# njspix/frender

Measured on AMD Instinct MI355X. Metric: M reads/sec scanned+classified (96 samples, 8+8bp, n=1) at 1/2/4/8 MI355X, higher is better.
Workload: dtype u8; 1 GPU; BASELINE config 2: 100000000 SYN-v1 reads/GPU, 96 samples, 8+8bp, n=1, R=8 (74 B/record), decoded FASTQ resident in HBM; reads_per_gpu=100000000, bytes_per_record=74, samples=96, nsubs=1, rc=False, unique_codes=1383958, table_checksum=a89b0e2c6adb2921, parallelism=1 GPU

## Files before the change

### frender_amd/csrc/fr_kernels.hip

```cpp
#include <algorithm>
#include <cstdlib>
#include <cstring>

#include <rocprim/rocprim.hpp>

#include "../../include/frender_amd.h"
#include "fr_internal.h"

namespace fr {

#if defined(FR_STAMPS) && FR_STAMPS == 1
#define FR_STAMP_DECL u64 st_[8] = {0, 0, 0, 0, 0, 0, 0, 0}; u64 tq_ = __builtin_amdgcn_s_memtime();
#define FR_STAMP(i) do { const u64 n_ = __builtin_amdgcn_s_memtime(); st_[i] += n_ - tq_; tq_ = n_; } while (0)
#define FR_STAMP_FLUSH(k0) do { st_[6] = __builtin_amdgcn_s_memtime() - (k0); \
    if ((threadIdx.x & 63) == 0) for (int i_ = 0; i_ < 8; ++i_) atomicAdd((unsigned long long*)&a.st->stamp[i_], \
        (unsigned long long)st_[i_]); } while (0)
#else
#define FR_STAMP_DECL
#define FR_STAMP(i) do { } while (0)
#define FR_STAMP_FLUSH(k0) do { } while (0)
#endif

#if defined(FR_STAMPS) && FR_STAMPS == 2
#define FR_CSTAMP(i) do { const u64 n_ = __builtin_amdgcn_s_memtime(); cst_[i] += n_ - cq_; cq_ = n_; } while (0)
#else
#define FR_CSTAMP(i) do { } while (0)
#endif

#if defined(FR_STAMPS) && FR_STAMPS == 4
#define FR_WSTAMP_DECL u64 wst_[4] = {0, 0, 0, 0}; u64 wq_ = __builtin_amdgcn_s_memtime();
#define FR_WSTAMP(i) do { const u64 n_ = __builtin_amdgcn_s_memtime(); wst_[i] += n_ - wq_; wq_ = n_; } while (0)
#define FR_WSTAMP_RESET() do { wq_ = __builtin_amdgcn_s_memtime(); } while (0)
#define FR_WSTAMP_FLUSH(steps) do { if ((threadIdx.x & 63) == 0) { \
    for (int i_ = 0; i_ < 4; ++i_) atomicAdd((unsigned long long*)&a.st->stamp[i_], (unsigned long long)wst_[i_]); \
    atomicAdd((unsigned long long*)&a.st->stamp[4], (unsigned long long)(steps)); \
    atomicAdd((unsigned long long*)&a.st->stamp[6], 1ull); } } while (0)
#else
#define FR_WSTAMP_DECL
#define FR_WSTAMP(i) do { } while (0)
#define FR_WSTAMP_RESET() do { } while (0)
#define FR_WSTAMP_FLUSH(steps) do { } while (0)
#endif

#ifdef FR_DEBUG_PRINT
#define FR_TRACE(...) do { if (blockIdx.x == 0 && (threadIdx.x & 63) == 0) printf(__VA_ARGS__); } while (0)
#else
#define FR_TRACE(...) do { } while (0)
#endif

#define FR_COLD __forceinline__

#ifndef FR_ABLATE
#define FR_ABLATE 0
#endif
constexpr u32 ABLATE = FR_ABLATE;


__device__ __forceinline__ u32 eq4(u32 w, u32 c) {
    const u32 t = w ^ c;
    const u32 z = ~(((t & 0x7F7F7F7Fu) + 0x7F7F7F7Fu) | t) & 0x80808080u;
    return (((z >> 7) * 0x00204081u) >> 21) & 0xFu;
}

__device__ __forceinline__ u32 hi4(u32 w) {
    return ((((w & 0x80808080u) >> 7) * 0x00204081u) >> 21) & 0xFu;
}

__device__ __forceinline__ u32 sym_of(u32 c) {
    const u32 i = (c >> 1) & 7u;
    const u64 expect = 0x4E002B0047544341ull;
    const u32 symtab = 0x50603421u;
    const bool ok = ((expect >> (8 * i)) & 0xFFu) == c;
    return ok ? ((symtab >> (4 * i)) & 0xFu) : 0u;
}

__device__ __forceinline__ u32 classify4(u32 w) {
    const u32 lo3 = __builtin_amdgcn_perm(0x10101310u, 0x10191014u, w & 0x07070707u);
    const u32 mid3 = __builtin_amdgcn_perm(0x18101014u, 0x10101310u, (w >> 3) & 0x07070707u);
    const u32 top2 = __builtin_amdgcn_perm(0u, 0x1010000Fu, (w >> 6) & 0x03030303u);
    return lo3 & mid3 & top2;
}

__device__ __forceinline__ u32 classify4_fast(u32 w) {
    const u32 lo3 = __builtin_amdgcn_perm(0x00008300u, 0x00890084u, w & 0x07070707u);
    const u32 hi4 = __builtin_amdgcn_perm(0x08000004u, 0x00000300u, (w >> 3) & 0x0F0F0F0Fu);
    return lo3 & hi4;
}

template <int K>
__device__ __forceinline__ u32 gather16(u32 c0, u32 c1, u32 c2, u32 c3) {
    constexpr u32 M = 0x01010101u << K;
    u32 v = __builtin_amdgcn_udot4(c0 & M, 0x08040201u, 0u, false);
    v = __builtin_amdgcn_udot4(c1 & M, 0x80402010u, v, false);
    u32 u = __builtin_amdgcn_udot4(c2 & M, 0x08040201u, 0u, false);
    u = __builtin_amdgcn_udot4(c3 & M, 0x80402010u, u, false);
    return (v | (u << 8)) >> K;
}

#ifndef FR_CLS_PAIR
#define FR_CLS_PAIR 1
#endif

constexpr u32 PAIR_CR = 0x04040404u, PAIR_SENTINEL = 0x40404040u;
__device__ __forceinline__ u32 classify8_pair(u32 wa, u32 wb) {
    const u32 lo_a = __builtin_amdgcn_perm(0x00004500u, 0x00430048u, wa & 0x87878787u);
    const u32 hi_a = __builtin_amdgcn_perm(0x02000008u, 0x00000500u, (wa >> 3) & 0x1F1F1F1Fu);
    const u32 lo_b = __builtin_amdgcn_perm(0x00005400u, 0x007000C0u, wb & 0x87878787u);
    const u32 hi_b = __builtin_amdgcn_perm(0x20000080u, 0x00001400u, (wb >> 3) & 0x1F1F1F1Fu);
    return __builtin_amdgcn_bitop3_b32(lo_a, hi_a, lo_b & hi_b, 0xEAu);
}

template <int K>
__device__ __forceinline__ u32 gather16p(u32 d0, u32 d1) {
    constexpr u32 M = 0x11111111u << K;
    const u32 v = __builtin_amdgcn_udot4(d0 & M, 0x08040201u, 0u, false);
    const u32 u = __builtin_amdgcn_udot4(d1 & M, 0x08040201u, 0u, false);
    return v | (u << 8);
}

template <int K>
__device__ __forceinline__ u64 join16p(const u32 (&g)[4]) {
    const u32 lo = (g[0] >> K) | (g[1] << (16 - K)), hi = (g[2] >> K) | (g[3] << (16 - K));
    return ((u64)hi << 32) | (u64)lo;
}

__device__ __forceinline__ u64 agent_load(const u64* p) {
    return __hip_atomic_load(p, __ATOMIC_RELAXED, __HIP_MEMORY_SCOPE_AGENT);
}
__device__ __forceinline__ void agent_store(u64* p, u64 v) {
    __hip_atomic_store(p, v, __ATOMIC_RELAXED, __HIP_MEMORY_SCOPE_AGENT);
}

__device__ __forceinline__ u64 wave_sum_u64(u64 v) {
#pragma unroll
    for (int d = 32; d >= 1; d >>= 1) v += __shfl_xor(v, d, 64);
    return v;
}

__device__ __forceinline__ u64 table_home(u64 key, u64 mask) {
    return mask ? mix64(key) >> __builtin_clzll(mask) : 0ull;
}

__device__ bool global_insert(const Table& T, DevState* st, u64 key, u64 cnt, u64 ord, u32 tag) {
    u64 h = table_home(key, T.mask);
    for (int probe = 0; probe < GPROBE; ++probe) {
        GSlot* s = &T.slots[h];
        const uint4 w0 = *(const uint4*)s;
        const uint4 w1 = *((const uint4*)s + 1);
        u64 k = ((u64)w0.y << 32) | w0.x;
        u64 first = ((u64)w1.y << 32) | w1.x;
        u32 ltag = w1.z;
        bool created = false;
        if (k == 0) {
            const u64 old = atomicCAS((unsigned long long*)&s->key, 0ull, (unsigned long long)key);
            created = old == 0;
            k = created ? key : old;
            first = ~0ull;
            ltag = 0;
        }
        if (k == key) {
            atomicAdd((unsigned long long*)&s->count, (unsigned long long)cnt);
            if (ord < first) atomicMin((unsigned long long*)&s->first, (unsigned long long)ord);
            if (ltag < tag) atomicMax(&s->last_tag, tag);
            return created;
        }
        h = (h + 1) & T.mask;
    }
    const u64 i = atomicAdd((unsigned long long*)&st->n_overflow, 1ull);
    if (i < T.ovf_cap) {
        Overflow o;
        o.key = key;
        o.count = cnt;
        o.first = ord;
        o.tag = tag;
        o.pad = 0;
        T.ovf[i] = o;
    } else {
        atomicOr(&st->cap_flags, 2u);
    }
    return false;
}

__device__ __forceinline__ void add_created(DevState* st, u32 mine) {
    u64 v = mine;
#pragma unroll
    for (int d = 32; d >= 1; d >>= 1) v += __shfl_xor(v, d, 64);
    if ((threadIdx.x & 63) == 0 && v) atomicAdd((unsigned long long*)&st->n_keys, (unsigned long long)v);
}

struct alignas(16) LSlot {
    u64 key;
    u32 cnt;
    u32 mino;
};

constexpr int NW = WG / 64;
constexpr int SEGS = TILE / SEG;
constexpr u32 RARE_WAVE = RARE_RING / NW;

struct ScanShared {
    u32 raw[NW][TILE / 4];
    LSlot ls[NS];
    u64 bsp[NW][SEGS + 2];
    u64 bcol[NW][SEGS + 2];
    u64 beol[NW][SEGS + 2];
    u64 wcount[NW];
    int wphase[NW];
    u32 rq_tail[NW];
    u64 tile_excl;
    u64 cbase;
    u32 chunk;
    u32 nkeys;
    u32 created;
    u32 flags;
    u32 last;
    u32 spec;
    u32 spec_bad;
    u32 ncold;
    u32 nexo;
    u32 err_off;
    u32 log_on;
    u32 exo_p[EXO_BUF], exo_start[EXO_BUF], exo_len[EXO_BUF];
};

typedef u32 u32x4 __attribute__((ext_vector_type(4)));
typedef __attribute__((address_space(3))) u32 lds_u32;
typedef __attribute__((address_space(3))) u32x4 lds_u32x4;
typedef __attribute__((address_space(3))) u64 lds_u64;
typedef __attribute__((address_space(3))) u8 lds_u8;

__device__ __forceinline__ u64 make_ord(const ScanArgs& a, u64 off_in_range) {
    return ((u64)a.file_tag << ORD_SHIFT) | ((a.file_offset + off_in_range) & ~3ull);
}

__device__ __forceinline__ u32 wave_id() { return __builtin_amdgcn_readfirstlane(threadIdx.x >> 6); }

__device__ __forceinline__ void lds_fence() {
    __builtin_amdgcn_fence(__ATOMIC_RELEASE, "workgroup", "local");
    __builtin_amdgcn_fence(__ATOMIC_ACQUIRE, "workgroup", "local");
}

__device__ __forceinline__ void lds_barrier() {
    __builtin_amdgcn_fence(__ATOMIC_RELEASE, "workgroup", "local");
    __builtin_amdgcn_s_barrier();
    __builtin_amdgcn_fence(__ATOMIC_ACQUIRE, "workgroup", "local");
}

__device__ FR_COLD void direct_insert(ScanShared& sh, const ScanArgs& a, u64 key, u32 off) {
    if (global_insert(a.tabv, a.st, key, 1, make_ord(a, sh.cbase + off), a.file_tag)) atomicAdd(&sh.created, 1u);
}

__device__ __forceinline__ void rare_push(ScanShared& sh, const ScanArgs& a, u32 p, u32 kind, u32 x, u32 y);

// ... 164 lines not shown
        if (c == '+') {
            if (plus != WIDE_NOPLUS) return false;
            plus = nl;
            continue;
        }
        const u32 lc = c | 0x20u;
        const int d = lc == 'a' ? 0 : lc == 'c' ? 1 : lc == 'g' ? 2 : lc == 't' ? 3 : lc == 'n' ? 4 : -1;
        if (d < 0 || nl >= WIDE_MAXN) return false;
        const int isl = (c & 0x20u) ? 1 : 0;
        if (lower < 0) lower = isl;
        else if (lower != isl) return false;
        v += (u64)d * pw;
        pw *= 5;
        ++nl;
    }
    if (lower < 0) return false;
    const int n1 = plus == WIDE_NOPLUS ? nl : plus, n2 = plus == WIDE_NOPLUS ? 0 : nl - plus;
    if (n1 > MAXSYM || n2 > MAXSYM) return false;
    key = WIDE_BIT | ((u64)lower << 62) | ((u64)plus << 57) | (v + (pw - 1) / 4);
    return true;
}

__device__ void exotic_record(const ScanArgs& a, u32 p, u64 start, u64 n, ScanShared& sh) {
    {
        bool fast = n >= 1 && n <= (u64)MAXSYM;
        u64 key = 0;
        for (u64 i = 0; fast && i < n; ++i) {
            const u32 sy = sym_of(a.buf[start + i]);
            fast = sy != 0;
            key |= (u64)sy << (3 * i);
        }
        if (fast || wide_encode(a, start, n, key)) {
            count_code<true>(sh, a, p, key);
            return;
        }
    }
    if (sh.spec) {
        const u32 k = atomicAdd(&sh.nexo, 1u);
        if (k < (u32)EXO_BUF) {
            sh.exo_p[k] = p;
            sh.exo_start[k] = (u32)(start - sh.cbase);
            sh.exo_len[k] = (u32)n;
        } else {
            atomicOr(&sh.spec_bad, 1u);
        }
        return;
    }
    const u64 i = atomicAdd((unsigned long long*)&a.st->n_exotic, 1ull);
    const u64 po = atomicAdd((unsigned long long*)&a.st->exo_pool_used, (unsigned long long)n);
    if (i < a.tabv.exo_cap && po + n <= a.tabv.exo_pool_cap) {
        a.tabv.exo_ord[i] = make_ord(a, sh.cbase + p);
        a.tabv.exo_off[i] = po;
        a.tabv.exo_len[i] = (u32)n;
        for (u64 k = 0; k < n; ++k) a.tabv.exo_pool[po + k] = a.buf[start + k];
    } else {
        atomicOr(&a.st->cap_flags, 4u);
    }
}

__device__ __forceinline__ void nospace(const ScanArgs& a, u32 p, ScanShared& sh) {
    if (sh.spec) atomicMin(&sh.err_off, p);
    else atomicMin((unsigned long long*)&a.st->err_nospace, (unsigned long long)(a.file_offset + sh.cbase + p));
}

__device__ FR_COLD void process_header_global(ScanShared& sh, const ScanArgs& a, u32 p) {
    const u64 eof = a.avail;
    auto rd = [&](u64 q) -> u32 { return (u32)a.buf[q]; };
    u64 q = sh.cbase + p;
    for (;;) {
        if (q >= eof) return nospace(a, p, sh);
        const u32 c = rd(q);
        if (c == ' ') break;
        if (c == '\n' || c == '\r') return nospace(a, p, sh);
        ++q;
    }
    const u64 sp1 = q++;
    i64 lc = -1;
    for (;;) {
        if (q >= eof) break;
        const u32 c = rd(q);
        if (c == ' ' || c == '\n' || c == '\r') break;
        if (c == ':') lc = (i64)q;
        ++q;
    }
    const u64 start = (lc >= 0 ? (u64)lc : sp1) + 1;
    const u64 n = q - start;
    u64 key = 0;
    bool fast = n >= 1 && n <= (u64)MAXSYM;
    for (u64 i = 0; fast && i < n; ++i) {
        const u32 sy = sym_of(rd(start + i));
        fast = sy != 0;
        key |= (u64)sy << (3 * i);
    }
    if (fast) count_code<true>(sh, a, p, key);
    else exotic_record(a, p, start, n, sh);
}

struct SegRegs {
    uint4 v[SEG / 16];
    u32 nx;
};

__device__ __forceinline__ void seg_fetch(const ScanArgs& a, u32 t, SegRegs& r, int lane, bool with_nx = false) {
    const u64 tile0 = (u64)t * TSTEP;
    const u32 nb = (u32)min((u64)TILE, a.avail - tile0);
    const u64 base = (u64)(a.buf + tile0);
    const u32 lo = __builtin_amdgcn_readfirstlane((u32)base), hi = __builtin_amdgcn_readfirstlane((u32)(base >> 32));
    const u8* ub = (const u8*)(((u64)hi << 32) | lo);
    const auto rsrc = __builtin_amdgcn_make_buffer_rsrc((void*)ub, (short)0, (int)__builtin_amdgcn_readfirstlane(nb),
                                                        0x00020000);
#pragma unroll
    for (int k = 0; k < SEG / 16; ++k) {
        const auto v = __builtin_amdgcn_raw_buffer_load_b128(rsrc, lane * SEG, k * 16, 0);
        r.v[k] = make_uint4(v[0], v[1], v[2], v[3]);
    }
    r.nx = with_nx ? __builtin_amdgcn_raw_buffer_load_b32(rsrc, lane * SEG + SEG, 0, 0) : 0u;
}

__device__ __attribute__((noinline)) SegRegs seg_load_tail(const ScanArgs& a, u32 t, int lane) {
    const u64 tile0 = (u64)t * TSTEP;
    const u32 nb = (u32)min((u64)TILE, a.avail - tile0);
    const u32 s0 = lane * SEG;
    u32 w[SEG / 4 + 1];
    for (int k = 0; k <= SEG / 4; ++k) {
        u32 v = 0;
        for (u32 q = 0; q < 4; ++q) {
            const u32 o = s0 + 4 * k + q;
            if (o < nb) v |= (u32)a.buf[tile0 + o] << (8 * q);
        }
        w[k] = v;
    }
    SegRegs r;
    for (int k = 0; k < SEG / 16; ++k) r.v[k] = make_uint4(w[4 * k], w[4 * k + 1], w[4 * k + 2], w[4 * k + 3]);
    r.nx = w[SEG / 4];
    return r;
}

__device__ __forceinline__ bool seg_in_range(const ScanArgs& a, u32 t) {
    return (u64)t * TSTEP + (TILE + SEG + 4) <= a.avail;
}

__device__ __forceinline__ void seg_load(const ScanArgs& a, u32 t, SegRegs& r, int lane) {
    if (seg_in_range(a, t)) seg_fetch(a, t, r, lane);
    else r = seg_load_tail(a, t, lane);
}

struct SegClass {
    u64 tmask, sp, col, eol;
    u32 c, x;
    u32 wtot;
    bool hi;
};

template <class Src>
__device__ __forceinline__ SegClass seg_classify_src(const ScanArgs& a, u32 t, const Src& src, int lane);

struct Cls16 {
    u32 eol[4], sp[4], col[4], acc;
};

__device__ __attribute__((noinline)) Cls16 classes_exact(const ScanArgs& a, u32 t, int lane) {
    SegRegs q;
    if (seg_in_range(a, t)) seg_fetch(a, t, q, lane);
    else q = seg_load_tail(a, t, lane);
    Cls16 r;
    r.acc = 0;
#pragma unroll
    for (int qv = 0; qv < SEG / 16; ++qv) {
        const u32 c0 = classify4(q.v[qv].x), c1 = classify4(q.v[qv].y), c2 = classify4(q.v[qv].z),
                  c3 = classify4(q.v[qv].w);
        r.eol[qv] = gather16<0>(c0, c1, c2, c3);
        r.sp[qv] = gather16<2>(c0, c1, c2, c3);
        r.col[qv] = gather16<3>(c0, c1, c2, c3);
        r.acc |= c0 | c1 | c2 | c3;
    }
    return r;
}

__device__ __forceinline__ SegClass seg_classify(const ScanArgs& a, u32 t, const SegRegs& r, int lane) {
    return seg_classify_src(a, t, [&](int k) { return r.v[k]; }, lane);
}

template <class Src>
__device__ __forceinline__ SegClass seg_classify_src(const ScanArgs& a, u32 t, const Src& src, int lane) {
    const u64 tile0 = (u64)t * TSTEP;
    const u32 tlen = (u32)min((u64)TSTEP, a.len - tile0);
    const u32 bl = (u32)min((u64)TILE, a.avail - tile0);
    const u32 s0 = lane * SEG;
    SegClass sc;
    sc.tmask = 0;
    sc.sp = sc.col = sc.eol = 0;
    sc.hi = false;
    if (s0 < bl) {
        u32 eol16[4], sp16[4], col16[4];
        u32 acc = 0;
        auto join = [](const u32 (&g)[4]) {
            return ((u64)(g[2] | (g[3] << 16)) << 32) | (u64)(g[0] | (g[1] << 16));
        };
#if FR_CLS_PAIR
#pragma unroll
        for (int qv = 0; qv < SEG / 16; ++qv) {
            const uint4 v = src(qv);
            const u32 d0 = classify8_pair(v.x, v.y), d1 = classify8_pair(v.z, v.w);
            eol16[qv] = gather16p<0>(d0, d1);
            col16[qv] = gather16p<1>(d0, d1);
            sp16[qv] = gather16p<3>(d0, d1);
            acc |= d0 | d1;
        }
        u64 eol = join16p<0>(eol16), sp = join16p<3>(sp16), col = join16p<1>(col16);
        bool cr = (acc & PAIR_CR) != 0;
        const bool slow = (acc & PAIR_SENTINEL) != 0;
#else
        u32 raw = 0;
#pragma unroll
        for (int qv = 0; qv < SEG / 16; ++qv) {
            const uint4 v = src(qv);
            const u32 c0 = classify4_fast(v.x), c1 = classify4_fast(v.y), c2 = classify4_fast(v.z),
                      c3 = classify4_fast(v.w);
            eol16[qv] = gather16<0>(c0, c1, c2, c3);
            sp16[qv] = gather16<2>(c0, c1, c2, c3);
            col16[qv] = gather16<3>(c0, c1, c2, c3);
            acc |= c0 | c1 | c2 | c3;
            raw |= v.x | v.y | v.z | v.w;
        }
        u64 eol = join(eol16), sp = join(sp16), col = join(col16);
        bool cr = (acc & 0x02020202u) != 0;
        const bool slow = ((acc | raw) & 0x80808080u) != 0;
#endif
        u32 hib = 0;
        if (__ballot(slow) != 0) {
            const Cls16 e = classes_exact(a, t, lane);
            eol = join(e.eol);
            sp = join(e.sp);
            col = join(e.col);
            cr = (e.acc & 0x02020202u) != 0;
            hib = e.acc & 0x10101010u;
        }
        u64 tm = eol;
        if (__ballot(cr) != 0) {
            SegRegs q;
            if (seg_in_range(a, t)) seg_fetch(a, t, q, lane, true);
            else q = seg_load_tail(a, t, lane);
            u32 cr16[4];
#pragma unroll
            for (int qv = 0; qv < SEG / 16; ++qv)
                cr16[qv] = gather16<1>(classify4(q.v[qv].x), classify4(q.v[qv].y), classify4(q.v[qv].z),
                                       classify4(q.v[qv].w));
            const u64 crm = join(cr16), nl = eol & ~crm;
            const u64 nxt = (q.nx & 0xFFu) == (u32)'\n' ? 1ull : 0ull;
            tm = eol & ~(crm & ((nl >> 1) | (nxt << 63)));
        }
        const u32 bvalid = bl - s0;
        if (bvalid < SEG) {
            const u64 vm = (1ull << bvalid) - 1ull;
            sp &= vm;
            col &= vm;
            eol &= vm;
        }
        if (s0 < tlen) {
            const u32 valid = tlen - s0;
            if (valid < SEG) tm &= (1ull << valid) - 1ull;
        } else {
            tm = 0;
        }
        sc.sp = sp;
        sc.col = col;
        sc.eol = eol;
        if (s0 < tlen) {
            sc.tmask = tm;
            sc.hi = hib != 0;
        }
    }
    sc.c = __popcll(sc.tmask);
    u32 x = sc.c;
    x += __builtin_amdgcn_update_dpp(0u, x, 0x111, 0xF, 0xF, true);
    x += __builtin_amdgcn_update_dpp(0u, x, 0x112, 0xF, 0xF, true);
    x += __builtin_amdgcn_update_dpp(0u, x, 0x114, 0xF, 0xF, true);
    x += __builtin_amdgcn_update_dpp(0u, x, 0x118, 0xF, 0xF, true);
    x += __builtin_amdgcn_update_dpp(0u, x, 0x142, 0xA, 0xF, false);
    x += __builtin_amdgcn_update_dpp(0u, x, 0x143, 0xC, 0xF, false);
    sc.x = x;
    sc.wtot = __builtin_amdgcn_readlane(x, 63);
    return sc;
}

__device__ FR_COLD void slow_header(ScanShared& sh, const ScanArgs& a, u32 p, int r, u32 start, u32 n);

__device__ __attribute__((noinline)) void drain_rare(ScanShared& sh, const ScanArgs& a, u32 wid, u32 from, u32 to,
                                                     int lane) {
    __builtin_amdgcn_fence(__ATOMIC_ACQ_REL, "workgroup");
    const uint4* q = a.rare + (u64)blockIdx.x * RARE_RING + wid * RARE_WAVE;
    for (u32 i = from + lane; i - from < to - from; i += 64) {
        const uint4 e = q[i & (RARE_WAVE - 1u)];
        if (e.y == 3u) {
            direct_insert(sh, a, ((u64)e.w << 32) | e.z, e.x);
        } else if (e.y == 4u) {
            const u64 x = sh.cbase + e.x;
            bool hi = false;
            for (u32 k = 0; k < e.z; ++k) hi |= a.buf[x + k] >= 0x80;
            if (hi) {
                atomicOr(&sh.flags, 1u);
                if (!utf8_segment_ok(a, x, e.z)) atomicOr(&sh.flags, 2u);
            }
        } else {
            slow_header(sh, a, e.x, (int)e.y, e.z, e.w);
        }
    }
}

__device__ __forceinline__ void seg_marks(const SegRegs& r, u64& at, u64& plus) {
    at = 0;
    plus = 0;
#pragma unroll
    for (int qv = 0; qv < SEG / 16; ++qv) {
        const u32 w[4] = {r.v[qv].x, r.v[qv].y, r.v[qv].z, r.v[qv].w};
#pragma unroll
        for (int k = 0; k < 4; ++k) {
            at |= (u64)eq4(w[k], 0x40404040u) << (qv * 16 + k * 4);
            plus |= (u64)eq4(w[k], 0x2B2B2B2Bu) << (qv * 16 + k * 4);
        }
    }
}

__device__ __forceinline__ int infer_phase(ScanShared& sh, const SegClass& sc, int lane, u32 wid) {
    lds_u32* E = (lds_u32*)&sh.raw[wid][0];
    u32 i = sc.x - sc.c;
    u64 m = sc.tmask;
    while (m && i <= (u32)PHASE_LINES) {
        E[i] = (u32)lane * SEG + (u32)__builtin_ctzll(m);
        m &= m - 1ull;
        ++i;
    }
    lds_fence();
    const u32 tot = __builtin_amdgcn_readlane(sc.x, 63);
    const int K = (int)min(tot, (u32)PHASE_LINES + 1u) - 1;
    if (K < 8) return -1;
    const bool valid = lane < K;
    int len = 0;
    bool is_at = false, is_plus = false;
    if (valid) {
// ... 341 lines not shown
            a.tabv.exo_off[i] = po;
            a.tabv.exo_len[i] = (u32)n;
            for (u64 q = 0; q < n; ++q) a.tabv.exo_pool[po + q] = a.buf[cb + sh.exo_start[k] + q];
        } else {
            atomicOr(&a.st->cap_flags, 4u);
        }
    }
    if (tid == 0 && sh.err_off != 0xFFFFFFFFu)
        atomicMin((unsigned long long*)&a.st->err_nospace, (unsigned long long)(a.file_offset + cb + sh.err_off));
    if (tid == 0) note_commit(a, g, hv);
    FR_CSTAMP(3);
    lds_barrier();
    FR_CSTAMP(4);
    for (int i = tid; i < NS; i += WG) sh.ls[i] = LSlot{0, 0, 0xFFFFFFFFu};
    if (tid == 0) {
        sh.nkeys = 0;
        sh.ncold = 0;
        sh.nexo = 0;
        sh.err_off = 0xFFFFFFFFu;
        sh.spec_bad = 0;
    }
    lds_barrier();
#if defined(FR_STAMPS) && FR_STAMPS == 2
    FR_CSTAMP(5);
    cst_[6] = nl;
    cst_[7] = nc;
    if ((tid & 63) == 0)
        for (int i_ = 0; i_ < 8; ++i_) atomicAdd((unsigned long long*)&a.st->stamp[i_], (unsigned long long)cst_[i_]);
#endif
}

__device__ __forceinline__ void discard_buffers(ScanShared& sh, int tid) {
    __syncthreads();
    for (int i = tid; i < NS; i += WG) sh.ls[i] = LSlot{0, 0, 0xFFFFFFFFu};
    if (tid == 0) {
        sh.nkeys = 0;
        sh.ncold = 0;
        sh.nexo = 0;
        sh.err_off = 0xFFFFFFFFu;
        sh.spec_bad = 0;
    }
    __syncthreads();
}

__device__ __forceinline__ bool uniform_flag(u32 v) { return __builtin_amdgcn_readfirstlane(v) != 0; }

__device__ __forceinline__ void encode_load_lds(const ScanShared& sh, u32 wid, u32 start, u32 (&w)[8]) {
    const lds_u32* p = (const lds_u32*)(&sh.raw[wid][0]) + (start >> 2);
#pragma unroll
    for (int k = 0; k < 8; ++k) w[k] = p[k];
}

__device__ __forceinline__ bool encode_pack(const u32 (&w)[8], u32 start, u32 n, u64& key) {
    if (n < 1 || n > (u32)MAXSYM) return false;
    const u32 sh = start & 3u;
    u64 kk = 0;
    u32 bad = 0;
#pragma unroll
    for (int k = 0; k < 6; ++k) {
        const u32 x = __builtin_amdgcn_alignbyte(w[k + 1], w[k], sh);
        const u32 idx = (x >> 1) & 0x07070707u;
        const u32 expect = __builtin_amdgcn_perm(0x4E002B00u, 0x47544341u, idx);
        const u32 sym = __builtin_amdgcn_perm(0x05000600u, 0x03040201u, idx);
        const int left = (int)n - 4 * k;
        const u32 vm = left >= 4 ? 0xFFFFFFFFu : left <= 0 ? 0u : (0xFFFFFFFFu >> (32 - 8 * left));
        bad |= (expect ^ x) & vm;
        const u32 sv = sym & vm;
        const u32 packed = __builtin_amdgcn_udot4(sv, 0x00400801u, (sv >> 15) & 0xE00u, false);
        kk |= (u64)packed << (12 * k);
    }
    key = kk;
    return bad == 0;
}

__device__ FR_COLD void slow_header(ScanShared& sh, const ScanArgs& a, u32 p, int r, u32 start, u32 n) {
    if (r == 2) process_header_global(sh, a, p);
    else if (r == 1) nospace(a, p, sh);
    else exotic_record(a, p, sh.cbase + start, n, sh);
}

__device__ __forceinline__ u32 ffbl32(u32 x) {
    u32 r;
    asm("v_ffbl_b32 %0, %1" : "=v"(r) : "v"(x));
    return r;
}
__device__ __forceinline__ u32 ffbh32(u32 x) {
    u32 r;
    asm("v_ffbh_u32 %0, %1" : "=v"(r) : "v"(x));
    return r;
}
__device__ __forceinline__ u32 ctz64x(u64 x) { return min(ffbl32((u32)x), ffbl32((u32)(x >> 32)) | 32u); }
__device__ __forceinline__ int hsb64x(u64 x) { return (int)(min(ffbh32((u32)(x >> 32)), ffbh32((u32)x) | 32u) ^ 63u); }

__device__ __forceinline__ u64 window64(u64 x0, u64 x1, u32 b) { return (x0 >> b) | ((x1 << 1) << (63u - b)); }

__device__ __forceinline__ int locate_code(const ScanShared& sh, u32 wid, u32 p, u32 bl, u32& start, u32& n) {
    const u32 w = min(p >> 6, (u32)SEGS - 1u), b = p & 63u;
    const lds_u64* S = (const lds_u64*)&sh.bsp[wid][w];
    const lds_u64* E = (const lds_u64*)&sh.beol[wid][w];
    const lds_u64* C = (const lds_u64*)&sh.bcol[wid][w];
    u64 s0 = S[0], s1 = S[1], s2 = S[2], e0 = E[0], e1 = E[1], c0 = C[0], c1 = C[1], c2 = C[2];
    asm volatile("" : "+v"(s0), "+v"(s1), "+v"(s2), "+v"(e0), "+v"(e1), "+v"(c0), "+v"(c1), "+v"(c2));
    if (p >= bl) return 2;
    const u64 se = window64(s0, s1, b);
    const u64 eo = window64(e0, e1, b);
    const u32 f1 = ctz64x(se);
    const u32 q = p + f1 + 1u;
    if (f1 >= 64u) return 2;
    if (ctz64x(eo) == f1) return 1;
    if (q >= bl) return 2;
    const bool nxt = (q >> 6) != w;
    const u32 b2 = q & 63u;
    const u64 se2 = window64(nxt ? s1 : s0, nxt ? s2 : s1, b2);
    const u64 co2 = window64(nxt ? c1 : c0, nxt ? c2 : c1, b2);
    const u32 f2 = ctz64x(se2);
    if (f2 >= 64u) return 2;
    const int hc = hsb64x(co2 & ((1ull << f2) - 1ull));
    const u32 cs = (u32)max(hc + 1, 0);
    start = q + cs;
    n = f2 - cs;
    return 0;
}

__device__ __forceinline__ bool encode_uniform(const ScanShared& sh, u32 wid, u32 start, u32 nu, u64& key) {
    u32 w[8];
    encode_load_lds(sh, wid, start, w);
    const u32 al = start & 3u;
    u32 bad = 0, lo = 0, hi = 0;
#pragma unroll
    for (int k = 0; k < 6; ++k) {
        if ((u32)(4 * k) >= nu) break;
        const u32 x = __builtin_amdgcn_alignbyte(w[k + 1], w[k], al);
        const u32 idx = (x >> 1) & 0x07070707u;
        const u32 expect = __builtin_amdgcn_perm(0x4E002B00u, 0x47544341u, idx);
        u32 sym = __builtin_amdgcn_perm(0x05000600u, 0x03040201u, idx);
        const u32 left = nu - 4u * k;
        if (left >= 4u) {
            bad |= expect ^ x;
        } else {
            const u32 vm = 0xFFFFFFFFu >> (32u - 8u * left);
            bad |= (expect ^ x) & vm;
            sym &= vm;
        }
        const u32 packed = __builtin_amdgcn_udot4(sym, 0x00400801u, (sym >> 15) & 0xE00u, false);
        if (k == 0) lo = packed;
        else if (k == 1) lo |= packed << 12;
        else if (k == 2) { lo |= packed << 24; hi = packed >> 8; }
        else hi |= packed << (12 * k - 32);
    }
    key = ((u64)hi << 32) | lo;
    return bad == 0;
}

__device__ __forceinline__ int locate_near(const ScanShared& sh, u32 wid, u32 p, u32 bl, u32& start, u32& n, u32& f1) {
    const u32 w = min(p >> 6, (u32)SEGS - 1u), b = p & 63u;
    const lds_u64* S = (const lds_u64*)&sh.bsp[wid][w];
    const lds_u64* C = (const lds_u64*)&sh.bcol[wid][w];
    u64 s0 = S[0], s1 = S[1], c0 = C[0], c1 = C[1];
    asm volatile("" : "+v"(s0), "+v"(s1), "+v"(c0), "+v"(c1));
    const u64 se = window64(s0, s1, b);
    const u64 co = window64(c0, c1, b);
    const u64 se1 = se & (se - 1ull);
    f1 = ctz64x(se);
    const u32 f2 = ctz64x(se1);
    const int hc = hsb64x(co & ((1ull << (f2 & 63u)) - 1ull));
    const u32 cs = (u32)max(hc, (int)f1) + 1u;
    start = p + cs;
    n = f2 - cs;
    return (p >= bl || se == 0ull) ? 2 : (se1 == 0ull ? 3 : 0);
}

__device__ __forceinline__ void parse_header(ScanShared& sh, const ScanArgs& a, u32 wid, u32 tile0, u32 p, u32 bl) {
    u32 start = 0, n = 0, f1 = 0;
    int r = locate_near(sh, wid, p, bl, start, n, f1);
    if (__ballot(r == 3) != 0) {
        if (r == 3) {
            r = locate_code(sh, wid, p, bl, start, n);
            f1 = 0xFFFFFFFFu;
        }
    }
    const u32 dch = *((const lds_u8*)&sh.raw[wid][0] + min(p + f1, (u32)TILE - 1u));
    if (ABLATE & 2u) {
        asm volatile("" ::"v"(start), "v"(n), "v"(r), "v"(dch));
        return;
    }
    u64 key = 0;
    bool fast = false;
    if (r == 0 && n >= 1u && n <= (u32)MAXSYM) {
        const u32 nu = __builtin_amdgcn_readfirstlane(n);
        if (__ballot(n != nu) == 0) {
            fast = encode_uniform(sh, wid, start, nu, key);
        } else {
            u32 w[8];
            encode_load_lds(sh, wid, start, w);
            fast = encode_pack(w, start, n, key);
        }
    }
    if (r == 0 && f1 < 64u && dch != (u32)' ') {
        r = 1;
        fast = false;
    }
    if (fast) count_code(sh, a, tile0 + p, key);
    else rare_push(sh, a, tile0 + p, (u32)r, tile0 + start, n);
}

template <bool LIM>
__device__ __forceinline__ void parse_own_headers(ScanShared& sh, const ScanArgs& a, u32 t, u32 ct,
                                                  const SegClass& sc, u64 L0, int lane, u32 wid) {
    const u64 tile0 = (u64)t * TSTEP;
    const u32 tile0c = (t - ct) * TSTEP;
    const u32 bl = (u32)min((u64)TILE, a.avail - tile0);
    const u64 rem64 = a.len - tile0;
    const u32 pend = rem64 >= 0xFFFFFFFFull ? 0xFFFFFFFFu : (u32)rem64 + ((a.own_end && a.len < a.avail) ? 1u : 0u);
    const u32 lb = (u32)L0 + (sc.x - sc.c);
    const u32 skip = (3u - lb) & 3u;
    const u32 s0 = lane * SEG;
    u64 m = sc.tmask;
#pragma unroll
    for (u32 q = 0; q < 3; ++q) {
        const u64 d = m & (m - 1ull);
        m = q < skip ? d : m;
    }
    constexpr bool limited = LIM;
    u64 rec = 0;
    if (limited) rec = (L0 + (sc.x - sc.c) + skip + 1u) >> 2;
    const bool own0s = t == 0 && a.own_start && (L0 & 3ull) == 0 && a.avail > 0 &&
                       (!limited || (i64)(L0 >> 2) < a.max_records);
    const bool own0 = own0s && lane == 0;
    const u32 p = own0 ? 0u : s0 + ctz64x(m) + 1u;
    const bool ok = own0 || (m != 0 && p < pend && (!limited || (i64)rec < a.max_records));
    if (ok) parse_header(sh, a, wid, tile0c, p, bl);
    bool more = ok && (own0 ? m != 0 : __popcll(m) > 4);
    if (!__ballot(more)) return;
    if (!own0) {
        m &= m - 1ull;
        m &= m - 1ull;
        m &= m - 1ull;
        m &= m - 1ull;
        ++rec;
    }
    while (__ballot(more)) {
        if (more) {
            const u32 pn = s0 + ctz64x(m) + 1u;
            more = pn < pend && (!limited || (i64)rec < a.max_records);
            if (more) parse_header(sh, a, wid, tile0c, pn, bl);
            ++rec;
            m &= m - 1ull;
            m &= m - 1ull;
            m &= m - 1ull;
            m &= m - 1ull;
            more = more && m != 0;
        }
    }
}

template <bool LIM>
__device__ __forceinline__ u64 walk_wave(ScanShared& sh, const ScanArgs& a0, u32 ct, u32 tb, u32 te, u64 L0,
                                         bool parse, int lane, u32 wid) {
    const ScanArgs& a = a0;
    u64 lines = 0;
    u32 done = *(const volatile lds_u32*)&sh.rq_tail[wid];
    SegRegs r;
    if (tb < te) seg_load(a, tb, r, lane);
    lds_u32x4* mine = (lds_u32x4*)(&sh.raw[wid][0]) + lane * (SEG / 16);
    FR_WSTAMP_DECL
    for (u32 t = tb; t < te; ++t) {
#if defined(FR_STAMPS) && FR_STAMPS == 4
        FR_WSTAMP_RESET();
        asm volatile("s_waitcnt vmcnt(0)" ::: "memory");
        FR_WSTAMP(0);
#endif
#pragma unroll
        for (int k = 0; k < SEG / 16; ++k) {
            u32x4 v;
            v.x = r.v[k].x; v.y = r.v[k].y; v.z = r.v[k].z; v.w = r.v[k].w;
            mine[k] = v;
        }
        if (t + 1 < te) seg_load(a, t + 1, r, lane);
        const SegClass sc = seg_classify_src(a, t, [&](int k) {
            const u32x4 v = *(const volatile lds_u32x4*)&mine[k];
            return make_uint4(v.x, v.y, v.z, v.w);
        }, lane);
        FR_WSTAMP(1);
        if (sc.hi) rare_push(sh, a, (t - ct) * TSTEP + lane * SEG, 4u,
                             min((u32)min((u64)TSTEP, a.len - (u64)t * TSTEP) - lane * SEG, (u32)SEG), 0u);
        const u32 tail = *(const volatile lds_u32*)&sh.rq_tail[wid];
        if (tail != done) {
            drain_rare(sh, a, wid, done, tail, lane);
            done = tail;
        }
        sh.bsp[wid][lane] = sc.sp | sc.eol;
        sh.bcol[wid][lane] = sc.col;
        sh.beol[wid][lane] = sc.eol;
        lds_fence();
        FR_WSTAMP(2);
        if (parse && !(ABLATE & 1u)) parse_own_headers<LIM>(sh, a, t, ct, sc, L0 + lines, lane, wid);
        lines += sc.wtot;
        FR_WSTAMP(3);
    }
    FR_WSTAMP_FLUSH(te > tb ? te - tb : 0u);
    lds_fence();
    const u32 tail = *(const volatile lds_u32*)&sh.rq_tail[wid];
    if (tail != done) drain_rare(sh, a, wid, done, tail, lane);
    return lines;
}

__device__ __forceinline__ u64 ramp_prefix(const Geom& g, u64 G, u64 j, u32 s0) {
    return ramp_tiles_before(g.chunk_tiles, G, s0, j);
}

__device__ __attribute__((noinline)) void verify_launch(ScanShared& sh, const ScanArgs& a, u32 n, u64 base_lines,
                                                       int tid) {
    const u32 per = (n + WG - 1) / WG;
    const u32 lo = min(tid * per, n), hi = min(lo + per, n);
    u64 sum = 0;
    for (u32 c = lo; c < hi; ++c) sum += (u32)agent_load(&a.chunk_info[c]);
    u64 x = sum;
    const int lane = tid & 63, wid = tid >> 6;
#pragma unroll
    for (int d = 1; d < 64; d <<= 1) {
        const u64 y = __shfl_up(x, d, 64);
        if (lane >= d) x += y;
    }
    if (lane == 63) sh.wcount[wid] = x;
    __syncthreads();
    u64 before = 0, total = 0;
#pragma unroll
    for (int w = 0; w < NW; ++w) {
        const u64 v = sh.wcount[w];
        before += w < wid ? v : 0ull;
        total += v;
    }
    u64 run = base_lines + before + (x - sum);
    bool bad = false;
    for (u32 c = lo; c < hi; ++c) {
        const u64 info = agent_load(&a.chunk_info[c]);
        const u32 f = (u32)(info >> 32);
        if ((f & 1u) && ((f >> 1) & 3u) != (u32)(run & 3ull)) bad = true;
        run += (u32)info;
    }
    if (bad) atomicOr(&a.st->spec_fail, 1u);
    if (tid == 0) a.st->lines[a.par ^ 1u] = base_lines + total;
    __syncthreads();
}

__device__ __forceinline__ void chunk_bounds(const ScanArgs& a, const Geom& g, u32 c, u32& tb, u32& te) {
    if (a.ramp_g == 0) {
        tb = min(c * g.chunk_tiles, a.num_tiles);
        te = min(tb + g.chunk_tiles, a.num_tiles);
        return;
    }
    const u32 su = min(a.ramp_up_s, g.chunk_tiles), sd = min(a.ramp_down_s, g.chunk_tiles);
    const u64 G = a.ramp_g, Gd = g.down_g;
    const u64 rg = ramp_prefix(g, G, G, su), mid_end = (u64)a.num_tiles - ramp_prefix(g, Gd, Gd, sd);
    if (c < G) {
        tb = (u32)ramp_prefix(g, G, c, su);
        te = (u32)ramp_prefix(g, G, c + 1, su);
    } else if (c < G + g.mid_chunks) {
        const u64 b = rg + (u64)(c - G) * g.chunk_tiles;
        tb = (u32)b;
        te = (u32)min(b + g.chunk_tiles, mid_end);
    } else {
        const u64 j = c - G - g.mid_chunks;
        tb = (u32)((u64)a.num_tiles - ramp_prefix(g, Gd, Gd - j, sd));
        te = (u32)((u64)a.num_tiles - ramp_prefix(g, Gd, Gd - j - 1, sd));
    }
}

#if defined(FR_STAMPS) && FR_STAMPS == 3
constexpr u32 TRACE_CHUNKS = 1u << 14;
constexpr u32 TRACE_WGS = 4096;
__device__ u64 g_chunk_trace[2 * TRACE_CHUNKS * 4];
__device__ u64 g_wg_trace[2 * TRACE_WGS * 2];
__device__ __forceinline__ u32 xcc_id() {
    u32 x;
    asm volatile("s_getreg_b32 %0, hwreg(HW_REG_XCC_ID)" : "=s"(x));
    return x & 0xFu;
}
extern "C" int fr_trace_read(u64* chunks, u64* wgs) {
    if (hipMemcpyFromSymbol(chunks, HIP_SYMBOL(g_chunk_trace), sizeof(g_chunk_trace)) != hipSuccess) return 1;
    if (hipMemcpyFromSymbol(wgs, HIP_SYMBOL(g_wg_trace), sizeof(g_wg_trace)) != hipSuccess) return 1;
    return 0;
}
extern "C" int fr_trace_clear() {
    static u64 zero[2 * TRACE_CHUNKS * 4];
    if (hipMemcpyToSymbol(HIP_SYMBOL(g_chunk_trace), zero, sizeof(g_chunk_trace)) != hipSuccess) return 1;
    if (hipMemcpyToSymbol(HIP_SYMBOL(g_wg_trace), zero, sizeof(g_wg_trace)) != hipSuccess) return 1;
    return 0;
}
#endif

#ifndef FR_OCC
#define FR_OCC 4
#endif
template <bool LIM>
__global__ __launch_bounds__(WG, FR_OCC) void chunk_kernel(ScanArgs args) {
    (void)args;
    const ScanArgs& a = *(const ScanArgs*)__builtin_amdgcn_kernarg_segment_ptr();
    __shared__ ScanShared sh;
    const int tid = threadIdx.x;
    const int lane = tid & 63;
    const u32 wid = wave_id();
    for (int i = tid; i < NS; i += WG) sh.ls[i] = LSlot{0, 0, 0xFFFFFFFFu};
    if (lane == 0) {
        sh.bsp[wid][SEGS] = sh.bsp[wid][SEGS + 1] = 0;
        sh.bcol[wid][SEGS] = sh.bcol[wid][SEGS + 1] = 0;
        sh.beol[wid][SEGS] = sh.beol[wid][SEGS + 1] = 0;
        sh.rq_tail[wid] = 0;
    }
    if (tid == 0) {
        sh.nkeys = 0;
        sh.created = 0;
        sh.flags = 0;
        sh.spec = 0;
        sh.spec_bad = 0;
        sh.ncold = 0;
        sh.nexo = 0;
        sh.err_off = 0xFFFFFFFFu;
        if (a.zero_fold && blockIdx.x == 0) a.st->log_fold_max = a.st->log_fold_over = 0;
    }
#if defined(FR_STAMPS) && FR_STAMPS == 3
    if (tid == 0 && blockIdx.x < TRACE_WGS) g_wg_trace[(a.par * TRACE_WGS + blockIdx.x) * 2] = __builtin_amdgcn_s_memrealtime();
    u64 tl_t0 = 0;
#endif
    const u64 base_lines = a.st->lines[a.par];
    const bool hv = a.num_chunks_h != 0 &&
                    __builtin_amdgcn_readfirstlane(__hip_atomic_load(&a.st->heavy[a.par], __ATOMIC_RELAXED,
                                                                     __HIP_MEMORY_SCOPE_AGENT)) != 0;
    const Geom g = hv ? Geom{a.chunk_tiles_h, a.mid_chunks_h, a.num_chunks_h, a.ramp_down_g_h}
                      : Geom{a.chunk_tiles, a.mid_chunks, a.num_chunks, a.ramp_down_g};
    constexpr bool limited = LIM;
#if defined(FR_STAMPS) && (FR_STAMPS == 1 || FR_STAMPS == 4)
    const u64 k0_ = __builtin_amdgcn_s_memtime();
#endif
    FR_STAMP_DECL
    for (;;) {
        if (tid == 0) {
            const u32 cn = atomicAdd(&a.st->ticket, 1u);
            sh.chunk = cn;
            if (cn < g.num_chunks) {
                u32 tb0, te0;
                chunk_bounds(a, g, cn, tb0, te0);
                sh.cbase = (u64)tb0 * TSTEP;
            }
            sh.spec = 1u;
        }
        __syncthreads();
        const u32 c = sh.chunk;
        FR_TRACE("w%d ticket %u of %u\n", (int)wid, c, g.num_chunks);
// ... 1040 lines not shown
```

Measured before the change: 41730 M reads/s.

## Locate headers from registers via DPP and use per-run buffer resource loads

The per-tile separator and colon bitmasks now stay in registers. Each lane gets its neighbour's words through a DPP lane shift, so headers are located without writing the bitmasks to LDS and fencing. The LDS arrays are filled lazily, and only when a header needs the far-locate fallback. Separately, the walk loop builds one buffer resource per run and uses 32-bit run-relative offsets, replacing the per-tile 64-bit address and bounds arithmetic. The risk is extra register pressure, and stale LDS bitmasks for any other consumer that expected them written every tile.

```diff
diff --git a/frender_amd/csrc/fr_kernels.hip b/frender_amd/csrc/fr_kernels.hip
--- a/frender_amd/csrc/fr_kernels.hip
+++ b/frender_amd/csrc/fr_kernels.hip
@@ -99,6 +99,13 @@
 
 #ifndef FR_CLS_PAIR
 #define FR_CLS_PAIR 1
+#endif
+
+#ifndef FR_HDR_REGS
+#define FR_HDR_REGS 1
+#endif
+#ifndef FR_WALK_CTX
+#define FR_WALK_CTX 1
 #endif
 
 constexpr u32 PAIR_CR = 0x04040404u, PAIR_SENTINEL = 0x40404040u;
@@ -569,8 +576,21 @@
     bool hi;
 };
 
+struct TileEnds {
+    u32 tlen, bl;
+};
+__device__ __forceinline__ TileEnds tile_ends(const ScanArgs& a, u32 t) {
+    const u64 tile0 = (u64)t * TSTEP;
+    return TileEnds{(u32)min((u64)TSTEP, a.len - tile0), (u32)min((u64)TILE, a.avail - tile0)};
+}
+
 template <class Src>
-__device__ __forceinline__ SegClass seg_classify_src(const ScanArgs& a, u32 t, const Src& src, int lane);
+__device__ __forceinline__ SegClass seg_classify_src(const ScanArgs& a, u32 t, const Src& src, int lane,
+                                                     const TileEnds& ends);
+template <class Src>
+__device__ __forceinline__ SegClass seg_classify_src(const ScanArgs& a, u32 t, const Src& src, int lane) {
+    return seg_classify_src(a, t, src, lane, tile_ends(a, t));
+}
 
 struct Cls16 {
     u32 eol[4], sp[4], col[4], acc;
@@ -599,10 +619,9 @@
 }
 
 template <class Src>
-__device__ __forceinline__ SegClass seg_classify_src(const ScanArgs& a, u32 t, const Src& src, int lane) {
-    const u64 tile0 = (u64)t * TSTEP;
-    const u32 tlen = (u32)min((u64)TSTEP, a.len - tile0);
-    const u32 bl = (u32)min((u64)TILE, a.avail - tile0);
+__device__ __forceinline__ SegClass seg_classify_src(const ScanArgs& a, u32 t, const Src& src, int lane,
+                                                     const TileEnds& ends) {
+    const u32 tlen = ends.tlen, bl = ends.bl;
     const u32 s0 = lane * SEG;
     SegClass sc;
     sc.tmask = 0;
@@ -1250,14 +1269,7 @@
     return bad == 0;
 }
 
-__device__ __forceinline__ int locate_near(const ScanShared& sh, u32 wid, u32 p, u32 bl, u32& start, u32& n, u32& f1) {
-    const u32 w = min(p >> 6, (u32)SEGS - 1u), b = p & 63u;
-    const lds_u64* S = (const lds_u64*)&sh.bsp[wid][w];
-    const lds_u64* C = (const lds_u64*)&sh.bcol[wid][w];
-    u64 s0 = S[0], s1 = S[1], c0 = C[0], c1 = C[1];
-    asm volatile("" : "+v"(s0), "+v"(s1), "+v"(c0), "+v"(c1));
-    const u64 se = window64(s0, s1, b);
-    const u64 co = window64(c0, c1, b);
+__device__ __forceinline__ int locate_in_windows(u64 se, u64 co, u32 p, u32 bl, u32& start, u32& n, u32& f1) {
     const u64 se1 = se & (se - 1ull);
     f1 = ctz64x(se);
     const u32 f2 = ctz64x(se1);
@@ -1268,15 +1280,69 @@
     return (p >= bl || se == 0ull) ? 2 : (se1 == 0ull ? 3 : 0);
 }
 
+__device__ __forceinline__ int locate_near(const ScanShared& sh, u32 wid, u32 p, u32 bl, u32& start, u32& n, u32& f1) {
+    const u32 w = min(p >> 6, (u32)SEGS - 1u), b = p & 63u;
+    const lds_u64* S = (const lds_u64*)&sh.bsp[wid][w];
+    const lds_u64* C = (const lds_u64*)&sh.bcol[wid][w];
+    u64 s0 = S[0], s1 = S[1], c0 = C[0], c1 = C[1];
+    asm volatile("" : "+v"(s0), "+v"(s1), "+v"(c0), "+v"(c1));
+    return locate_in_windows(window64(s0, s1, b), window64(c0, c1, b), p, bl, start, n, f1);
+}
+
+struct HdrWords {
+    u64 sp, col;
+    u64 nsp, ncol;
+};
+
+__device__ __forceinline__ u64 window_own(u64 own, u64 next, u32 b) {
+    const u64 lo = b < 64u ? own >> (b & 63u) : 0ull;
+    const u64 hi = b != 0u ? next << ((64u - b) & 63u) : 0ull;
+    return lo | hi;
+}
+
+__device__ __forceinline__ int locate_near_regs(const HdrWords& hw, u32 b, u32 p, u32 bl, u32& start, u32& n, u32& f1) {
+    return locate_in_windows(window_own(hw.sp, hw.nsp, b), window_own(hw.col, hw.ncol, b), p, bl, start, n, f1);
+}
+
+__device__ __forceinline__ void finish_header(ScanShared& sh, const ScanArgs& a, u32 wid, u32 tile0, u32 p, u32 bl,
+                                              int r, u32 start, u32 n, u32 f1);
+
+__device__ __forceinline__ void locate_far(const ScanShared& sh, u32 wid, u32 p, u32 bl, int& r, u32& start, u32& n,
+                                           u32& f1) {
+    if (r == 3) {
+        r = locate_code(sh, wid, p, bl, start, n);
+        f1 = 0xFFFFFFFFu;
+    }
+}
+
+__device__ __forceinline__ void header_step(ScanShared& sh, const ScanArgs& a, u32 wid, u32 tile0, bool ok, u32 p,
+                                            u32 b, u32 bl, const HdrWords& hw, u64 eol, int lane, bool& staged) {
+    u32 start = 0, n = 0, f1 = 0;
+    int r = locate_near_regs(hw, b, p, bl, start, n, f1);
+    if (__ballot(ok && r == 3) != 0) {
+        if (!staged) {
+            sh.bsp[wid][lane] = hw.sp;
+            sh.bcol[wid][lane] = hw.col;
+            sh.beol[wid][lane] = eol;
+            lds_fence();
+            staged = true;
+        }
+        if (ok) locate_far(sh, wid, p, bl, r, start, n, f1);
+    }
+    if (ok) finish_header(sh, a, wid, tile0, p, bl, r, start, n, f1);
+}
+
 __device__ __forceinline__ void parse_header(ScanShared& sh, const ScanArgs& a, u32 wid, u32 tile0, u32 p, u32 bl) {
     u32 start = 0, n = 0, f1 = 0;
     int r = locate_near(sh, wid, p, bl, start, n, f1);
     if (__ballot(r == 3) != 0) {
-        if (r == 3) {
-            r = locate_code(sh, wid, p, bl, start, n);
-            f1 = 0xFFFFFFFFu;
-        }
-    }
+        locate_far(sh, wid, p, bl, r, start, n, f1);
+    }
+    finish_header(sh, a, wid, tile0, p, bl, r, start, n, f1);
+}
+
+__device__ __forceinline__ void finish_header(ScanShared& sh, const ScanArgs& a, u32 wid, u32 tile0, u32 p, u32 bl,
+                                              int r, u32 start, u32 n, u32 f1) {
     const u32 dch = *((const lds_u8*)&sh.raw[wid][0] + min(p + f1, (u32)TILE - 1u));
     if (ABLATE & 2u) {
         asm volatile("" ::"v"(start), "v"(n), "v"(r), "v"(dch));
@@ -1304,12 +1370,9 @@
 
 template <bool LIM>
 __device__ __forceinline__ void parse_own_headers(ScanShared& sh, const ScanArgs& a, u32 t, u32 ct,
-                                                  const SegClass& sc, u64 L0, int lane, u32 wid) {
-    const u64 tile0 = (u64)t * TSTEP;
+                                                  const SegClass& sc, u64 L0, int lane, u32 wid, u32 bl, u32 pend,
+                                                  const HdrWords& hw) {
     const u32 tile0c = (t - ct) * TSTEP;
-    const u32 bl = (u32)min((u64)TILE, a.avail - tile0);
-    const u64 rem64 = a.len - tile0;
-    const u32 pend = rem64 >= 0xFFFFFFFFull ? 0xFFFFFFFFu : (u32)rem64 + ((a.own_end && a.len < a.avail) ? 1u : 0u);
     const u32 lb = (u32)L0 + (sc.x - sc.c);
     const u32 skip = (3u - lb) & 3u;
     const u32 s0 = lane * SEG;
@@ -1327,7 +1390,12 @@
     const bool own0 = own0s && lane == 0;
     const u32 p = own0 ? 0u : s0 + ctz64x(m) + 1u;
     const bool ok = own0 || (m != 0 && p < pend && (!limited || (i64)rec < a.max_records));
+#if FR_HDR_REGS
+    bool staged = false;
+    if (__ballot(ok)) header_step(sh, a, wid, tile0c, ok, p, p - s0, bl, hw, sc.eol, lane, staged);
+#else
     if (ok) parse_header(sh, a, wid, tile0c, p, bl);
+#endif
     bool more = ok && (own0 ? m != 0 : __popcll(m) > 4);
     if (!__ballot(more)) return;
     if (!own0) {
@@ -1338,6 +1406,17 @@
         ++rec;
     }
     while (__ballot(more)) {
+#if FR_HDR_REGS
+        const u32 pn = s0 + ctz64x(m) + 1u;
+        more = more && pn < pend && (!limited || (i64)rec < a.max_records);
+        header_step(sh, a, wid, tile0c, more, pn, pn - s0, bl, hw, sc.eol, lane, staged);
+        ++rec;
+        m &= m - 1ull;
+        m &= m - 1ull;
+        m &= m - 1ull;
+        m &= m - 1ull;
+        more = more && m != 0;
+#else
         if (more) {
             const u32 pn = s0 + ctz64x(m) + 1u;
             more = pn < pend && (!limited || (i64)rec < a.max_records);
@@ -1349,6 +1428,7 @@
             m &= m - 1ull;
             more = more && m != 0;
         }
+#endif
     }
 }
 
@@ -1359,7 +1439,31 @@
     u64 lines = 0;
     u32 done = *(const volatile lds_u32*)&sh.rq_tail[wid];
     SegRegs r;
+#if FR_WALK_CTX
+    const u64 run0 = (u64)tb * TSTEP;
+    const u32 availr = __builtin_amdgcn_readfirstlane((u32)min(a.avail - run0, (u64)0x7FFFFFFFu));
+    const u32 lenr = __builtin_amdgcn_readfirstlane((u32)min(a.len - run0, (u64)0x7FFFFFFFu));
+    const u32 pend_x = (a.own_end && a.len < a.avail) ? 1u : 0u;
+    const u64 rbase = (u64)(a.buf + run0);
+    const u32 rlo = __builtin_amdgcn_readfirstlane((u32)rbase), rhi = __builtin_amdgcn_readfirstlane((u32)(rbase >> 32));
+    const auto rsrc = __builtin_amdgcn_make_buffer_rsrc((void*)(((u64)rhi << 32) | rlo), (short)0, (int)availr, 0x00020000);
+    auto in_range = [&](u32 o) { return o + (u32)(TILE + SEG + 4) <= availr; };
+    auto fetch = [&](u32 o) {
+#pragma unroll
+        for (int k = 0; k < SEG / 16; ++k) {
+            const auto v = __builtin_amdgcn_raw_buffer_load_b128(rsrc, lane * SEG, (int)(o + k * 16), 0);
+            r.v[k] = make_uint4(v[0], v[1], v[2], v[3]);
+        }
+        r.nx = 0u;
+    };
+    if (tb < te) {
+        if (in_range(0u)) fetch(0u);
+        else r = seg_load_tail(a, tb, lane);
+    }
+    u32 so = 0;
+#else
     if (tb < te) seg_load(a, tb, r, lane);
+#endif
     lds_u32x4* mine = (lds_u32x4*)(&sh.raw[wid][0]) + lane * (SEG / 16);
     FR_WSTAMP_DECL
     for (u32 t = tb; t < te; ++t) {
@@ -1374,25 +1478,51 @@
             v.x = r.v[k].x; v.y = r.v[k].y; v.z = r.v[k].z; v.w = r.v[k].w;
             mine[k] = v;
         }
+#if FR_WALK_CTX
+        if (t + 1 < te) {
+            if (in_range(so + (u32)TSTEP)) fetch(so + (u32)TSTEP);
+            else r = seg_load_tail(a, t + 1, lane);
+        }
+        const TileEnds ends{min((u32)TSTEP, lenr - so), min((u32)TILE, availr - so)};
+        const u32 pend = lenr - so + pend_x;
+        so += (u32)TSTEP;
+#else
         if (t + 1 < te) seg_load(a, t + 1, r, lane);
+        const TileEnds ends = tile_ends(a, t);
+        const u64 rem64 = a.len - (u64)t * TSTEP;
+        const u32 pend = rem64 >= 0xFFFFFFFFull ? 0xFFFFFFFFu : (u32)rem64 + ((a.own_end && a.len < a.avail) ? 1u : 0u);
+#endif
         const SegClass sc = seg_classify_src(a, t, [&](int k) {
             const u32x4 v = *(const volatile lds_u32x4*)&mine[k];
             return make_uint4(v.x, v.y, v.z, v.w);
-        }, lane);
+        }, lane, ends);
         FR_WSTAMP(1);
-        if (sc.hi) rare_push(sh, a, (t - ct) * TSTEP + lane * SEG, 4u,
-                             min((u32)min((u64)TSTEP, a.len - (u64)t * TSTEP) - lane * SEG, (u32)SEG), 0u);
+        if (sc.hi) rare_push(sh, a, (t - ct) * TSTEP + lane * SEG, 4u, min(ends.tlen - lane * SEG, (u32)SEG), 0u);
         const u32 tail = *(const volatile lds_u32*)&sh.rq_tail[wid];
         if (tail != done) {
             drain_rare(sh, a, wid, done, tail, lane);
             done = tail;
         }
-        sh.bsp[wid][lane] = sc.sp | sc.eol;
+        HdrWords hw;
+        hw.sp = sc.sp | sc.eol;
+        hw.col = sc.col;
+#if FR_HDR_REGS
+        auto next_lane = [](u64 x) {
+            const u32 lo = __builtin_amdgcn_update_dpp(0u, (u32)x, 0x130, 0xF, 0xF, false);
+            const u32 hi = __builtin_amdgcn_update_dpp(0u, (u32)(x >> 32), 0x130, 0xF, 0xF, false);
+            return ((u64)hi << 32) | lo;
+        };
+        hw.nsp = next_lane(hw.sp);
+        hw.ncol = next_lane(hw.col);
+#else
+        hw.nsp = hw.ncol = 0;
+        sh.bsp[wid][lane] = hw.sp;
         sh.bcol[wid][lane] = sc.col;
         sh.beol[wid][lane] = sc.eol;
         lds_fence();
+#endif
         FR_WSTAMP(2);
-        if (parse && !(ABLATE & 1u)) parse_own_headers<LIM>(sh, a, t, ct, sc, L0 + lines, lane, wid);
+        if (parse && !(ABLATE & 1u)) parse_own_headers<LIM>(sh, a, t, ct, sc, L0 + lines, lane, wid, ends.bl, pend, hw);
         lines += sc.wtot;
         FR_WSTAMP(3);
     }
```

Measured after the change: 42050 M reads/s (median of 6 runs). No clear change (+0.8%).
